# talha-alam/ADAM-Dehaze

Measured on AMD Instinct MI355X. Metric: images/sec CORUN-Complex fwd+bwd 512x1024 bs=8; PSNR vs CPU ref, higher is better.
Workload: dtype f32; 1 GPU; CORUN-Complex (HighIntensityDehazeModel base 96) train-mode fwd + L1 + bwd + Adam; per_gpu_batch=8, global_batch=8, height=512, width=1024, parallelism=dp1

## Files before the change

adam-dehaze_amd/csrc/conv_wino43.hip:

```cpp
#include "common.h"
#ifndef W_STORE_AUX
#define W_STORE_AUX 0
#endif
#include <cstdlib>
#include <type_traits>

#ifndef W4_DBG
#define W4_DBG 0
#endif
#ifndef W4_STORE_NOPS
#define W4_STORE_NOPS 1
#endif
#define W4_KC 16
#define W4_ZERO_C false
#define W4_TILES 32
#define W4_VF (36 * W4_TILES * W4_KC)
#define W4_SLOTS 612
#define W4_ROWSLOTS 34
#define W4_RAWF (40 * 256)
#define W4_TAB (W4_VF + W4_RAWF)
#define W4_TABF (4 * 640)
#define W4_MF (36 * 16 * 32)
#define W4_RED (W4_TAB + 3 * W4_TABF)
#define W4_LDS_BYTES ((W4_RED + 2 * 8 * 32) * 4)
static_assert(W4_MF <= W4_VF, "the epilogue's M must not reach the raw halo: the next region's first chunk lands there meanwhile");
#ifndef W4_P2
#define W4_P2 0
#endif
#define W4_PIECE_G0 2

#define W4B_RAW_B 73728
#define W4B_RAWBUF_B 40960
#define W4B_TAB_B 155648
#define W4B_LDS_BYTES (W4B_TAB_B + 3 * 2560)
static_assert(W4B_LDS_BYTES <= 160 * 1024, "LDS map of the bf16 x 3 variant");
#define B3_NO_SPLIT ((W4_DBG & 16) != 0)
#include "bf16x3.h"

typedef __attribute__((address_space(3))) void* lds_void_ptr4;

#ifdef W4_PROF
__device__ unsigned long long w4_prof_buf[16384 * 32];
#define W4_STAMP(i) do { if (tid == 0 && v < 16384) w4_prof_buf[v * 32 + (i)] = __builtin_readcyclecounter(); } while (0)
extern "C" int adh_w4_prof_read(void* dst) {
    return hipMemcpyFromSymbol(dst, HIP_SYMBOL(w4_prof_buf), sizeof(w4_prof_buf)) == hipSuccess ? 0 : -1;
}
#else
#define W4_STAMP(i) do {} while (0)
#endif

struct Wino43Geom {
    int tiles_x, tiles_y;
    int nregions;
    int nchunks;
    int KQtot;
    int ncog;
    int nvblocks;
    unsigned m_ncog, m_tx, m_ty;
    const float* bn_mean;
};

template <int NT, int FI, int J>
constexpr bool w4_in_agpr() {
    constexpr int nv = 9 * NT - 16;
    if constexpr (nv <= 0) return true;
    else if constexpr (nv <= 9) return !(J == 0 && FI >= 9 - nv);
    else return !(J == 0 || (J == 1 && FI >= 9 - (nv - 9)));
}
template <bool AGPR, bool Z = false>
__device__ __forceinline__ void w4_mfma(f32x16& c, float a, float b) {
    if constexpr (Z) {
        if constexpr (AGPR) asm("v_mfma_f32_32x32x2_f32 %0, %1, %2, 0" : "+a"(c) : "v"(a), "v"(b));
        else asm("v_mfma_f32_32x32x2_f32 %0, %1, %2, 0" : "+v"(c) : "v"(a), "v"(b));
    } else {
        if constexpr (AGPR) asm("v_mfma_f32_32x32x2_f32 %0, %1, %2, %0" : "+a"(c) : "v"(a), "v"(b));
        else asm("v_mfma_f32_32x32x2_f32 %0, %1, %2, %0" : "+v"(c) : "v"(a), "v"(b));
    }
}
#ifndef W4_MFMA_ZERO
#define W4_MFMA_ZERO 1
#endif
template <int NT, int T = 0>
__device__ __forceinline__ void w4_acc_zero_(f32x16 (&acc)[9 * NT], const u32x4& z) {
    if constexpr (T < 9 * NT) {
        if constexpr (w4_in_agpr<NT, T / NT, T % NT>()) asm volatile("v_mfma_f32_32x32x16_bf16 %0, %1, %1, 0" : "=a"(acc[T]) : "v"(z));
        else asm volatile("v_mfma_f32_32x32x16_bf16 %0, %1, %1, 0" : "=&v"(acc[T]) : "v"(z));
        w4_acc_zero_<NT, T + 1>(acc, z);
    }
}
template <int NT>
__device__ __forceinline__ void w4_acc_zero(f32x16 (&acc)[9 * NT]) {
    u32x4 z = {0u, 0u, 0u, 0u};
    asm volatile("s_nop 1" : "+v"(z));
    w4_acc_zero_<NT>(acc, z);
// ... 461 lines not shown
            in_next = image_ptr(wn.n);
            tab_nxt = tab_base;
            if (wn.border) {
                tab_nxt = tab_base + (1 + (tsel ^ 1)) * TABN;
                build_table(tab_nxt, wn.oy0, wn.ox0, false);
            }
        }
        W4_STAMP(4);
        const float* const b_wave = d.wp + ((int64_t)(wave * 9) * g.KQtot * d.NcP + co0) * 4;
        const char* const b3_wave = reinterpret_cast<const char*>(d.wp) + ((size_t)cg * g.nchunks * 36 + (size_t)wave * 9) * (NT * 3072);
        if constexpr (!BF3) {
            w4_load_b<NT>(bv[0], b_voff, b_wave);
            w4_load_b<NT>(bv[1], b_voff, b_wave + b_fstride);
        }
        W4_STAMP(5);
#if W4_MFMA_ZERO
        w4_acc_zero<NT>(acc);
#else
#pragma unroll
        for (int t = 0; t < 9 * NT; ++t)
#pragma unroll
            for (int r = 0; r < 16; ++r) acc[t][r] = 0.f;
#endif
        if (it == 0) asm volatile("s_waitcnt vmcnt(0)" ::: "memory");
        asm volatile("s_waitcnt lgkmcnt(0)" ::: "memory");
        __builtin_amdgcn_s_barrier();

        W4_STAMP(1);
#pragma unroll 1
        for (int c = 0; c < g.nchunks; ++c) {
            const bool more = c + 1 < g.nchunks;
            const bool cross = !more && has_next;
            st.cb = __builtin_amdgcn_readfirstlane((more ? (c + 1) * (W4_KC * 4) : (cross ? 0 : c * (W4_KC * 4))) + (cross ? wn.base : wc.base));
            st.rsrc = image_rsrc(cross ? in_next : in_cur);
            const int* const stab = cross ? tab_nxt : tab_cur;
            st.tab_lane = stab + tab_lane_o;
            if (c == 1) W4_STAMP(8);
            if (c == 1) W4_STAMP(9);
            if (!(W4_DBG & 1)) transform(cpar, stab);
            asm volatile("s_waitcnt lgkmcnt(0)" ::: "memory");
            if (c == 1) W4_STAMP(10);
            if constexpr (BF3) {
                if (!(W4_DBG & 2)) {
                    w4b_load_b(bv3[0], b3_voff, b3_wave + c * b3_cstride);
                    w4b_load_b(bv3[1], b3_voff, b3_wave + c * b3_cstride + 3072);
                }
            }
            __builtin_amdgcn_s_barrier();
            if (c == 1) W4_STAMP(11);
            if constexpr (BF3) {
                if (!(W4_DBG & 2)) {
                    w4b_load_s(nx, vlane, vlane1);
                    w4b_steps<0, 20>(nx, m1s);
                    av3[0] = u32x4{nx.h[0], nx.h[1], nx.h[2], nx.h[3]};
                    av3[1] = u32x4{nx.m[0], nx.m[1], nx.m[2], nx.m[3]};
                    av3[2] = u32x4{nx.l[0], nx.l[1], nx.l[2], nx.l[3]};
                    asm volatile("s_nop 1" : "+v"(av3[0]), "+v"(av3[1]), "+v"(av3[2]));
                    w4b_load_s(nx, vlane + W4_TILES * W4_KC, vlane1 + W4_TILES * W4_KC);
                    __builtin_amdgcn_sched_barrier(0);
                    w4b_groups<NT, 0, W4_ZERO_C>(acc, av3, nx, bv3, vlane, vlane1, b3_voff, b3_wave + c * b3_cstride, m1s);
                }
            } else if (!(W4_DBG & 2)) {
                const int cn = more ? c + 1 : c;
                const float* b_chunk = b_wave + (int64_t)(c * 4) * b_kq;
                const float* b_next = b_wave + (int64_t)(cn * 4) * b_kq;
                w4_contract<NT, W4_ZERO_C>(acc, av, bv, vlane, vlane1, b_voff, b_chunk, b_next, b_fstride, b_kq, st);
            }
            if (c == 1) W4_STAMP(12);
            cpar ^= 1;
            asm volatile("s_waitcnt lgkmcnt(0)" ::: "memory");
            __builtin_amdgcn_s_barrier();
            if (c == 1) W4_STAMP(13);
        }
        if constexpr (!BF3) {
            w4_wait_b<0, NT>(bv[0]);
            w4_wait_b<0, NT>(bv[1]);
        } else {
            asm volatile("s_waitcnt vmcnt(0)" ::: "memory");
        }
        W4_STAMP(2);

        if (!(W4_DBG & 4)) {
            float* M = lds;
            const int etp = (tid >> 3) & 15, eq = tid & 7;
            const int rh = wave >> 1;
            const int et = (etp & 8) | ((etp & 1) << 2) | ((etp >> 1) & 3);
            const int ey0 = oy0 + 4 * (et >> 3) + 2 * rh, ex0 = ox0 + 4 * (et & 7);
            float* out_n = d.out + (size_t)n * d.OH * d.OW * d.out_cstride;
            const float* res_n = d.residual ? d.residual + (size_t)n * d.OH * d.OW * d.res_cstride : nullptr;
            const int o_px = d.out_cstride * 4, o_row = d.OW * o_px;
            const int r_px = d.res_cstride * 4, r_row = d.OW * r_px;
            const __amdgpu_buffer_rsrc_t orsrc = __builtin_amdgcn_make_buffer_rsrc(out_n, 0, 0x7fffffff, 0x00020000);
            const __amdgpu_buffer_rsrc_t rrsrc =
                __builtin_amdgcn_make_buffer_rsrc(const_cast<float*>(res_n ? res_n : out_n), 0, 0x7fffffff, 0x00020000);
            const bool ragged = oy0 + 16 > d.OH || ox0 + 32 > d.OW;
            const float act_lo = d.act == ADH_ACT_RELU ? 0.f : -INFINITY;
            unsigned colpen[4];
#pragma unroll
            for (int r = 0; r < 4; ++r) colpen[r] = ex0 + r < d.OW ? 0u : 0x80000000u;
            const unsigned o_vbase = (unsigned)((ey0 * d.OW + ex0) * o_px + (co0 + eq * 4) * 4);
            const unsigned r_vbase = (unsigned)((ey0 * d.OW + ex0) * r_px + (co0 + eq * 4) * 4);
            const unsigned m_wbase = (unsigned)((wave * 9) * 2048 + h * 128 + l31 * 4);
            const float* const mp = M + etp * 32 + eq * 4;
            const float m1 = adh_opaque(-1.f);
            float* const red = BF3 ? lds + RAW0 + (cpar ^ 1) * (W4B_RAWBUF_B / 4) : lds + W4_RED;
            typedef unsigned u32x4 __attribute__((ext_vector_type(4)));
            w4_store_mh<NT, 0>(acc, m_wbase, 0);
            asm volatile("s_waitcnt lgkmcnt(0)" ::: "memory");
            __builtin_amdgcn_s_barrier();
#pragma unroll
            for (int j = 0; j < NT; ++j) {
                const int cq0 = co0 + j * 32 + eq * 4;
                const bool quad_ok = cq0 + 3 < d.Cout;
                f32x4 sc4 = {1.f, 1.f, 1.f, 1.f}, sh4 = {0.f, 0.f, 0.f, 0.f};
                if (d.scale && quad_ok) sc4 = *reinterpret_cast<const f32x4*>(d.scale + cq0);
                if (d.shift && quad_ok) sh4 = *reinterpret_cast<const f32x4*>(d.shift + cq0);
                f32x4 mean4 = {0.f, 0.f, 0.f, 0.f};
                if constexpr (BNRED) {
                    if (quad_ok) mean4 = *reinterpret_cast<const f32x4*>(g.bn_mean + cq0);
                }
                const unsigned chanpen = quad_ok ? 0u : 0x80000000u;
                const unsigned o_vj = (o_vbase + j * 128) | chanpen, r_vj = (r_vbase + j * 128) | chanpen;
                f32x4 ssum = {0.f, 0.f, 0.f, 0.f}, ssq = {0.f, 0.f, 0.f, 0.f};
#pragma unroll
                for (int th = 0; th < 2; ++th) {
                    if (j == 1 && th == 0) W4_STAMP(16);
                    f32x4 u[2][6];
#pragma unroll
                    for (int b = 0; b < 6; ++b) {
                        f32x4 m[6];
#pragma unroll
                        for (int a = 0; a < 6; ++a) m[a] = *reinterpret_cast<const f32x4*>(mp + (a * 6 + b) * (16 * 32));
                        const f32x4 s12 = m[1] + m[2], d12 = adh_pksub(m[1], m[2], m1), s34 = m[3] + m[4], d34 = adh_pksub(m[3], m[4], m1);
                        if (rh == 0) {
                            u[0][b] = m[0] + s12 + s34;
                            u[1][b] = W4_A * d12 + W4_B * d34;
                        } else {
                            u[0][b] = W4_A2 * s12 + W4_B2 * s34;
                            u[1][b] = W4_A3 * d12 + W4_B3 * d34 + m[5];
                        }
                    }
                    if (j == 1 && th == 0) W4_STAMP(17);
                    __builtin_amdgcn_s_barrier();
                    if (j == 1 && th == 0) W4_STAMP(18);
                    const int jn = th == 0 ? j : j + 1, thn = th ^ 1;
                    w4_store_mh_round<NT>(acc, m_wbase, jn, thn, 0);
                    if (j == 1 && th == 0) W4_STAMP(19);
                    unsigned rowpen[2];
#pragma unroll
                    for (int r = 0; r < 2; ++r) rowpen[r] = ey0 + 8 * th + r < d.OH ? 0u : 0x80000000u;
                    f32x4 rres[8];
                    if (res_n) {
#pragma unroll
                        for (int ii = 0; ii < 2; ++ii)
#pragma unroll
                            for (int jj = 0; jj < 4; ++jj)
                                rres[ii * 4 + jj] = __builtin_bit_cast(
                                    f32x4, __builtin_amdgcn_raw_buffer_load_b128(rrsrc, r_vj | rowpen[ii] | colpen[jj],
                                                                                 (8 * th + ii) * r_row + jj * r_px, 0));
                        asm volatile("" ::: "memory");
                    } else {
#pragma unroll
                        for (int q = 0; q < 8; ++q) rres[q] = f32x4{0.f, 0.f, 0.f, 0.f};
                    }
#pragma unroll
                    for (int ii = 0; ii < 2; ++ii) {
                        const f32x4 s12 = u[ii][1] + u[ii][2], d12 = adh_pksub(u[ii][1], u[ii][2], m1), s34 = u[ii][3] + u[ii][4],
                                    d34 = adh_pksub(u[ii][3], u[ii][4], m1);
                        const f32x4 y[4] = {u[ii][0] + s12 + s34, W4_A * d12 + W4_B * d34, W4_A2 * s12 + W4_B2 * s34,
                                            W4_A3 * d12 + W4_B3 * d34 + u[ii][5]};
#pragma unroll
                        for (int jj = 0; jj < 4; ++jj) {
                            const unsigned oaddr = o_vj | rowpen[ii] | colpen[jj];
                            if constexpr (BNRED) {
                                const f32x4 yv = rres[ii * 4 + jj];
                                const bool inside = (int)oaddr >= 0;
                                f32x4 gm;
#pragma unroll
                                for (int e = 0; e < 4; ++e) gm[e] = (inside && __builtin_fmaf(yv[e], sc4[e], sh4[e]) > 0.f) ? y[jj][e] : 0.f;
                                ssum += gm;
                                ssq += gm * adh_pksub(yv, mean4, m1);
                                f32x4 v4 = y[jj];
                                __builtin_amdgcn_raw_buffer_store_b128(__builtin_bit_cast(u32x4, v4), orsrc, oaddr,
                                                                       (8 * th + ii) * o_row + jj * o_px, W_STORE_AUX);
                                asm volatile("s_nop %1" : "+v"(v4) : "n"(W4_STORE_NOPS) : "memory");
                                w4_store_mh_round<NT>(acc, m_wbase, jn, thn, 1 + ii * 4 + jj);
                                continue;
                            }
                            f32x4 v4 = y[jj] * sc4 + sh4;
                            if (d.stats) {
                                f32x4 vs = v4;
                                if (ragged) {
                                    const bool inside = (int)oaddr >= 0;
#pragma unroll
                                    for (int e = 0; e < 4; ++e) vs[e] = inside ? v4[e] : 0.f;
                                    asm volatile("" : "+v"(vs));
                                }
                                ssum += vs;
                                ssq += vs * vs;
                            }
                            v4 += rres[ii * 4 + jj];
                            v4 = {fmaxf(v4[0], act_lo), fmaxf(v4[1], act_lo), fmaxf(v4[2], act_lo), fmaxf(v4[3], act_lo)};
                            __builtin_amdgcn_raw_buffer_store_b128(__builtin_bit_cast(u32x4, v4), orsrc, oaddr, (8 * th + ii) * o_row + jj * o_px,
                                                                   W_STORE_AUX);
                            asm volatile("s_nop %1" : "+v"(v4) : "n"(W4_STORE_NOPS) : "memory");
                            w4_store_mh_round<NT>(acc, m_wbase, jn, thn, 1 + ii * 4 + jj);
                        }
                    }
                    if (j == 1 && th == 0) W4_STAMP(20);
                    if (!(j == NT - 1 && th == 1)) {
                        asm volatile("s_waitcnt lgkmcnt(0)" ::: "memory");
                        __builtin_amdgcn_s_barrier();
                    }
                    if (j == 1 && th == 0) W4_STAMP(21);
                }
                if (d.stats) {
#pragma unroll
                    for (int e = 0; e < 4; ++e) {
#pragma unroll
                        for (int o = 8; o < 64; o <<= 1) {
                            ssum[e] += __shfl_xor(ssum[e], o, 64);
                            ssq[e] += __shfl_xor(ssq[e], o, 64);
                        }
                    }
// ... 287 lines not shown
```

adam-dehaze_amd/csrc/cbam.hip:

```cpp
#include "common.h"

#ifndef POOL_PPB
#define POOL_PPB 512
#endif
#ifndef CBAM_SCALE_MAXBLK
#define CBAM_SCALE_MAXBLK 65536
#endif
#ifndef CBAM_ROW_MAXBLK
#define CBAM_ROW_MAXBLK 2048
#endif

extern "C" int adh_cbam_pool_num_blocks(int HW) { return adh_ceil_div(HW, POOL_PPB); }

__global__ __launch_bounds__(256) void cbam_pool_partial_kernel(const float* __restrict__ x, int x_cs, int HW, int C,
                                                                float* __restrict__ partial,
                                                                int32_t* __restrict__ partial_idx, int nblk) {
    __shared__ f32x4 rs[256];
    __shared__ f32x4 rm[256];
    __shared__ int ri[256][4];
    const int n = blockIdx.y, blk = blockIdx.x;
    const int CQ = C / 4;
    const int R = 256 / CQ;
    const int cq = threadIdx.x % CQ, prow = threadIdx.x / CQ;
    const int c = cq * 4;
// ... 240 lines not shown
        sa[((size_t)n * H + y) * W + x] = 1.0f / (1.0f + expf(-v));
    }
}

__global__ __launch_bounds__(256) void cbam_scale_kernel(const float* __restrict__ x, int x_cs, const float* __restrict__ ca,
                                                         const float* __restrict__ sa, int64_t HW, int CQ,
                                                         float* __restrict__ out, int out_cs) {
    const int n = blockIdx.y;
    int64_t p, pstep;
    int c;
    adh_stream_decode(CQ, p, pstep, c);
    const f32x4 cav = *reinterpret_cast<const f32x4*>(ca + (size_t)n * CQ * 4 + c);
    const float* xn = x + (size_t)n * HW * x_cs;
    float* on = out + (size_t)n * HW * out_cs;
    const float* san = sa + (size_t)n * HW;
    for (; p < HW; p += 8 * pstep) {
        f32x4 v[8];
        float sv[8];
#pragma unroll
        for (int u = 0; u < 8; ++u) {
            const int64_t q = p + u * pstep < HW ? p + u * pstep : p;
            v[u] = __builtin_nontemporal_load(reinterpret_cast<const f32x4*>(xn + q * x_cs + c));
            sv[u] = san[q];
        }
#pragma unroll
        for (int u = 0; u < 8; ++u) {
            const int64_t q = p + u * pstep;
            if (q < HW) __builtin_nontemporal_store(v[u] * cav * sv[u], reinterpret_cast<f32x4*>(on + q * out_cs + c));
        }
    }
}

extern "C" int adh_cbam_apply(void* stream, const float* x, int x_cs, const float* ca, const float* smap,
                              const float* wsp, int N, int H, int W, int C, float* sa, float* out, int out_cs) {
    if (!x || !ca || !smap || !wsp || !sa || !out || N < 1 || H < 1 || W < 1 || C < 4 || (C & 3) || (x_cs & 3) || (out_cs & 3) ||
        N > 65535)
        return ADH_E_ARG;
    hipStream_t s = (hipStream_t)stream;
    hipLaunchKernelGGL(cbam_sa_kernel, dim3(adh_ceil_div(W, SA_TW), adh_ceil_div(H, SA_TH), N), dim3(256), 0, s, smap, wsp, H, W,
                       sa);
    hipLaunchKernelGGL(cbam_scale_kernel, dim3(adh_stream_blocks((int64_t)H * W, C / 4, 8, CBAM_SCALE_MAXBLK), N), dim3(256), 0, s,
                       x, x_cs, ca, sa, (int64_t)H * W, C / 4, out, out_cs);
    return adh_check_launch();
}

__global__ __launch_bounds__(256) void cbam_bwd_a_kernel(const float* __restrict__ g, int g_cs,
                                                         const float* __restrict__ x, int x_cs,
                                                         const float* __restrict__ ca, const float* __restrict__ sa,
                                                         int HW, int C, float* __restrict__ gsa_pre) {
    const int n = blockIdx.y;
    const int sub = threadIdx.x & 7;
    const int CQ = C / 4;
    const float* xn = x + (size_t)n * HW * x_cs;
    const float* gn = g + (size_t)n * HW * g_cs;
    const float* can = ca + (size_t)n * C;
    for (int p = blockIdx.x * 32 + (threadIdx.x >> 3); p < HW; p += gridDim.x * 32) {
        float s = 0.f;
        for (int q = sub; q < CQ; q += 8) {
            const f32x4 v = __builtin_nontemporal_load(reinterpret_cast<const f32x4*>(xn + (size_t)p * x_cs + q * 4)) *
                            *reinterpret_cast<const f32x4*>(can + q * 4) *
                            __builtin_nontemporal_load(reinterpret_cast<const f32x4*>(gn + (size_t)p * g_cs + q * 4));
            s += (v[0] + v[1]) + (v[2] + v[3]);
        }
#pragma unroll
        for (int o = 4; o > 0; o >>= 1) s += __shfl_xor(s, o, 64);
        if (sub == 0) {
            const float a = sa[(size_t)n * HW + p];
            gsa_pre[(size_t)n * HW + p] = s * a * (1.f - a);
        }
    }
}

extern "C" int adh_cbam_bwd_a(void* stream, const float* g, int g_cs, const float* x, int x_cs, const float* ca,
                              const float* sa, int N, int HW, int C, float* gsa_pre) {
    if (!g || !x || !ca || !sa || !gsa_pre || N < 1 || HW < 1 || C < 4 || (C & 3)) return ADH_E_ARG;
    const int blocks = adh_min_i(adh_ceil_div(HW, 32), CBAM_ROW_MAXBLK);
    hipLaunchKernelGGL(cbam_bwd_a_kernel, dim3(blocks, N), dim3(256), 0, (hipStream_t)stream, g, g_cs, x, x_cs, ca, sa, HW,
                       C, gsa_pre);
    return adh_check_launch();
}

extern "C" int adh_cbam_bwd_b_num_blocks(int N, int H, int W) { return adh_ceil_div((int64_t)N * H * W, 256); }

__global__ __launch_bounds__(256) void cbam_bwd_b_kernel(const float* __restrict__ gsa_pre,
                                                         const float* __restrict__ smap, const float* __restrict__ wsp,
                                                         int N, int H, int W, float* __restrict__ gsmap,
                                                         float* __restrict__ dwsp_partial) {
    __shared__ float s_w[98];
    __shared__ float s_acc[4][98];
    if (threadIdx.x < 98) s_w[threadIdx.x] = wsp[threadIdx.x];
    __syncthreads();
    const int64_t total = (int64_t)N * H * W;
    const int64_t idx = (int64_t)blockIdx.x * 256 + threadIdx.x;
    const bool valid = idx < total;
    int n = 0, y = 0, xx = 0;
    if (valid) {
        xx = (int)(idx % W);
        const int64_t r = idx / W;
        y = (int)(r % H);
        n = (int)(r / H);
    }
    const float* gp = gsa_pre + (size_t)n * H * W;
    const float* sm = smap + (size_t)n * H * W * 2;
    const float gs_here = valid ? gp[(size_t)y * W + xx] : 0.f;
    float g0 = 0.f, g1 = 0.f;
    const int wave = threadIdx.x >> 6, lane = threadIdx.x & 63;
    for (int ky = 0; ky < 7; ++ky) {
        for (int kx = 0; kx < 7; ++kx) {
            const int oy = y - ky + 3, ox = xx - kx + 3;
            if (valid && oy >= 0 && oy < H && ox >= 0 && ox < W) {
                const float go = gp[(size_t)oy * W + ox];
                g0 += go * s_w[ky * 7 + kx];
                g1 += go * s_w[49 + ky * 7 + kx];
            }
            const int iy = y + ky - 3, ix = xx + kx - 3;
            float a0 = 0.f, a1 = 0.f;
            if (valid && iy >= 0 && iy < H && ix >= 0 && ix < W) {
                const float* q = sm + ((size_t)iy * W + ix) * 2;
                a0 = q[0] * gs_here;
                a1 = q[1] * gs_here;
            }
            a0 = wave_sum(a0);
            a1 = wave_sum(a1);
            if (lane == 0) {
                s_acc[wave][ky * 7 + kx] = a0;
                s_acc[wave][49 + ky * 7 + kx] = a1;
            }
        }
    }
    if (valid) {
        gsmap[idx * 2 + 0] = g0;
        gsmap[idx * 2 + 1] = g1;
    }
    __syncthreads();
    if (threadIdx.x < 98)
        dwsp_partial[(size_t)blockIdx.x * 98 + threadIdx.x] =
            (s_acc[0][threadIdx.x] + s_acc[1][threadIdx.x]) + (s_acc[2][threadIdx.x] + s_acc[3][threadIdx.x]);
}

__global__ __launch_bounds__(256) void cbam_dwsp_final_kernel(const float* __restrict__ partial, int nblk, float* dwsp,
                                                              int accumulate) {
    __shared__ double red[256];
    const int o = blockIdx.x;
    double s = 0.0;
    for (int b = threadIdx.x; b < nblk; b += 256) s += (double)partial[(size_t)b * 98 + o];
    red[threadIdx.x] = s;
    __syncthreads();
    for (int st = 128; st > 0; st >>= 1) {
        if (threadIdx.x < st) red[threadIdx.x] += red[threadIdx.x + st];
        __syncthreads();
    }
    if (threadIdx.x == 0) dwsp[o] = accumulate ? dwsp[o] + (float)red[0] : (float)red[0];
}

extern "C" int adh_cbam_bwd_b(void* stream, const float* gsa_pre, const float* smap, const float* wsp, int N, int H,
                              int W, float* gsmap, float* dwsp_partial, int nblk, float* dwsp, int accumulate) {
    if (!gsa_pre || !smap || !wsp || !gsmap || !dwsp_partial || !dwsp) return ADH_E_ARG;
    if (nblk != adh_cbam_bwd_b_num_blocks(N, H, W)) return ADH_E_ARG;
    hipStream_t s = (hipStream_t)stream;
    hipLaunchKernelGGL(cbam_bwd_b_kernel, dim3(nblk), dim3(256), 0, s, gsa_pre, smap, wsp, N, H, W, gsmap, dwsp_partial);
    hipLaunchKernelGGL(cbam_dwsp_final_kernel, dim3(98), dim3(256), 0, s, dwsp_partial, nblk, dwsp, accumulate);
    return adh_check_launch();
}

__device__ __forceinline__ f32x4 cbam_gx1(const f32x4 g, float sa, float gmean_over_c, float gmax, int cidx, int c) {
    f32x4 r = g * sa + gmean_over_c;
#pragma unroll
    for (int j = 0; j < 4; ++j)
        if (c + j == cidx) r[j] += gmax;
    return r;
}

__global__ __launch_bounds__(256) void cbam_bwd_c_kernel(const float* __restrict__ g, int g_cs,
                                                         const float* __restrict__ x, int x_cs,
                                                         const float* __restrict__ sa, const float* __restrict__ gsmap,
                                                         const int32_t* __restrict__ cidx, int HW, int C,
                                                         float* __restrict__ gca_partial, int nblk) {
    __shared__ f32x4 rs[256];
    const int n = blockIdx.y, blk = blockIdx.x;
    const int CQ = C / 4;
    const int R = 256 / CQ;
    const int cq = threadIdx.x % CQ, prow = threadIdx.x / CQ;
    const int c = cq * 4;
    const float invC = 1.0f / (float)C;
    f32x4 s = {0.f, 0.f, 0.f, 0.f};
    if (prow < R) {
        const float* xn = x + (size_t)n * HW * x_cs;
        const float* gn = g + (size_t)n * HW * g_cs;
        const int p0 = blk * POOL_PPB;
        const int p1 = adh_min_i(p0 + POOL_PPB, HW);
        for (int p = p0 + prow; p < p1; p += 4 * R) {
            f32x4 gv[4], xv[4];
            float sv[4], gm[4], gx[4];
            int ci[4];
#pragma unroll
            for (int u = 0; u < 4; ++u) {
                const int q = p + u * R < p1 ? p + u * R : p;
                const size_t pp = (size_t)n * HW + q;
                gv[u] = __builtin_nontemporal_load(reinterpret_cast<const f32x4*>(gn + (size_t)q * g_cs + c));
                xv[u] = __builtin_nontemporal_load(reinterpret_cast<const f32x4*>(xn + (size_t)q * x_cs + c));
                sv[u] = sa[pp];
                gm[u] = gsmap[pp * 2 + 0];
                gx[u] = gsmap[pp * 2 + 1];
                ci[u] = cidx[pp];
            }
#pragma unroll
            for (int u = 0; u < 4; ++u)
                if (p + u * R < p1) s += cbam_gx1(gv[u], sv[u], gm[u] * invC, gx[u], ci[u], c) * xv[u];
        }
    }
    rs[threadIdx.x] = s;
    __syncthreads();
    if (threadIdx.x < CQ) {
        f32x4 S = {0.f, 0.f, 0.f, 0.f};
        for (int r = 0; r < R; ++r) S += rs[r * CQ + threadIdx.x];
        *reinterpret_cast<f32x4*>(gca_partial + ((size_t)n * nblk + blk) * C + c) = S;
    }
}

extern "C" int adh_cbam_bwd_c(void* stream, const float* g, int g_cs, const float* x, int x_cs, const float* sa,
                              const float* gsmap, const int32_t* cidx, int N, int HW, int C, float* gca_partial,
                              int nblk) {
    if (!g || !x || !sa || !gsmap || !cidx || !gca_partial || C < 4 || (C & 3) || C > 1024) return ADH_E_ARG;
    if (nblk != adh_cbam_pool_num_blocks(HW)) return ADH_E_ARG;
    hipLaunchKernelGGL(cbam_bwd_c_kernel, dim3(nblk, N), dim3(256), 0, (hipStream_t)stream, g, g_cs, x, x_cs, sa, gsmap,
                       cidx, HW, C, gca_partial, nblk);
    return adh_check_launch();
}

__global__ __launch_bounds__(256) void cbam_bwd_d1_kernel(const float* __restrict__ gca_partial, int nblk,
                                                          const float* __restrict__ ca, int C, float* __restrict__ gpre) {
    __shared__ double red[8][32];
    const int n = blockIdx.y;
    const int cl = threadIdx.x & 31, grp = threadIdx.x >> 5;
    const int c = blockIdx.x * 32 + cl;
    double s = 0.0;
    if (c < C)
        for (int b = grp; b < nblk; b += 8) s += (double)gca_partial[((size_t)n * nblk + b) * C + c];
    red[grp][cl] = s;
    __syncthreads();
    if (grp == 0 && c < C) {
// ... 145 lines not shown
```

adam-dehaze_amd/csrc/conv_wgrad.hip:

```cpp
#include "common.h"
#include <cstdlib>

#define WG_TW 32

template <int T, int TN>
__global__ __launch_bounds__(512, 2) void conv_wgrad_kernel(const adh_conv_desc d, const ConvGeom g, float* slab,
                                                            int ntiles, int KP, int nco_groups) {
    extern __shared__ __attribute__((aligned(16))) float smem[];
    constexpr int BN = 32 * TN;
    constexpr int PER = (T * TN + 3) / 4;
    const int XP = g.xp;
    const int buf_floats = g.npx * XP + 32 + g.TH * WG_TW * BN;

    const int tid = threadIdx.x;
    const int lane = tid & 63;
    const int wave = __builtin_amdgcn_readfirstlane(tid >> 6);
    const bool loader = wave >= 4;
    const int l31 = lane & 31;
    const int h = lane >> 5;

    const int ci_tile = blockIdx.x / nco_groups;
    const int co_grp = blockIdx.x - ci_tile * nco_groups;
    const int ci0 = ci_tile * 32;
    const int co0 = co_grp * BN;
// ... 528 lines not shown
                p.a.xps = 2;
                p.a.ymin = d->dy0 + py;
                p.a.xmin = d->dx0 + px;
                p.a.tap0 = py * 4 + px; p.a.tap_sy = 8; p.a.tap_sx = 2;
            }
        return 4;
    }
    return 0;
}

template <int KH, int KW, bool REV, int TN>
static int launch_wgrad_rows(hipStream_t s, const adh_conv_desc* d, const WrArgs& a, float* slab) {
    const int lds = 2 * (((WR_TH + KH - 1) * WR_HP + TN * WR_TH * 32) * 32 * 4);
    const int nblocks = adh_split_grid_blocks(a.nsplit, a.ngroups);
    (void)hipFuncSetAttribute(reinterpret_cast<const void*>(&conv_wgrad_rows_kernel<KH, KW, REV, TN>),
                              hipFuncAttributeMaxDynamicSharedMemorySize, 160 * 1024);
    hipLaunchKernelGGL((conv_wgrad_rows_kernel<KH, KW, REV, TN>), dim3(nblocks), dim3(256), lds, s, *d, a, slab);
    return adh_check_launch();
}

static int dispatch_wgrad_rows(hipStream_t s, const adh_conv_desc* d, const WrPlan& p, float* slab) {
#define WR_CASE(kh_, kw_, rev_, tn_) \
    if (p.KH == kh_ && p.KW == kw_ && p.rev == rev_ && p.TN == tn_) \
        return launch_wgrad_rows<kh_, kw_, rev_ != 0, tn_>(s, d, p.a, slab);
    WR_CASE(3, 3, 0, 3) WR_CASE(3, 3, 0, 2) WR_CASE(3, 3, 0, 1)
    WR_CASE(2, 2, 0, 3) WR_CASE(2, 2, 0, 2) WR_CASE(2, 2, 0, 1)
    WR_CASE(2, 2, 1, 3) WR_CASE(2, 2, 1, 2) WR_CASE(2, 2, 1, 1)
#undef WR_CASE
    return ADH_E_UNSUPPORTED;
}

static bool wgrad_rows_instantiated(const WrPlan& p) {
    return (p.KH == 3 && p.KW == 3 && !p.rev) || (p.KH == 2 && p.KW == 2);
}

static int wgrad_wino_plan(const adh_conv_desc* d, int nsplit, WrPlan* p) {
    static const bool enabled = !(getenv("ADH_WINO_WGRAD") && atoi(getenv("ADH_WINO_WGRAD")) == 0);
    if (!enabled) return 0;
    WrPlan plan[4];
    if (wgrad_rows_plan(d, nsplit, plan) != 1) return 0;
    if (plan[0].KH != 3 || plan[0].KW != 3 || plan[0].rev || plan[0].a.xps != 1) return 0;
    if (d->dy0 != -1 || d->dx0 != -1) return 0;
    *p = plan[0];
    return 1;
}

extern "C" int adh_conv_wgrad_wino_groups(const adh_conv_desc* d) {
    if (!d) return ADH_E_ARG;
    WrPlan p;
    return wgrad_wino_plan(d, 1, &p) ? p.a.ngroups : 0;
}

extern "C" int adh_conv_wgrad_wino(void* stream, const adh_conv_desc* d, float* slab, int nsplit) {
    if (!d || !slab || nsplit < 1 || !d->in || !d->out) return ADH_E_ARG;
    WrPlan p;
    if (!wgrad_wino_plan(d, nsplit, &p)) return ADH_E_UNSUPPORTED;
    const int lds = 2 * (((WR_TH + 2) * WR_HP + p.TN * WR_TH * 32) * 32 * 4);
    const int nblocks = adh_split_grid_blocks(nsplit, p.a.ngroups);
    hipStream_t s = (hipStream_t)stream;
#define WW_CASE(tn_) \
    if (p.TN == tn_) { \
        (void)hipFuncSetAttribute(reinterpret_cast<const void*>(&conv_wgrad_rows_kernel<3, 3, false, tn_, true>), \
                                  hipFuncAttributeMaxDynamicSharedMemorySize, 160 * 1024); \
        hipLaunchKernelGGL((conv_wgrad_rows_kernel<3, 3, false, tn_, true>), dim3(nblocks), dim3(256), lds, s, *d, p.a, slab); \
        return adh_check_launch(); \
    }
    WW_CASE(3) WW_CASE(2) WW_CASE(1)
#undef WW_CASE
    return ADH_E_UNSUPPORTED;
}

extern "C" int adh_conv_wgrad_groups(const adh_conv_desc* d) {
    if (!d) return ADH_E_ARG;
    WrPlan plan[4];
    const int n = wgrad_rows_plan(d, 1, plan);
    return n && wgrad_rows_instantiated(plan[0]) ? plan[0].a.ngroups : 0;
}

extern "C" int adh_conv_wgrad_slabs(const adh_conv_desc* d, int nsplit) {
    if (!d || nsplit < 1) return ADH_E_ARG;
    return adh_conv_wgrad_groups(d) > 0 ? 4 * nsplit : nsplit;
}

extern "C" int adh_conv_wgrad(void* stream, const adh_conv_desc* d, float* slab, int nsplit) {
    if (!d || !slab || nsplit < 1 || !d->in || !d->out) return ADH_E_ARG;
    if (d->NcP % 32 != 0 || d->NcP < d->Cout) return ADH_E_ARG;
    {
        WrPlan plan[4];
        const int np = wgrad_rows_plan(d, nsplit, plan);
        if (np && wgrad_rows_instantiated(plan[0])) {
            for (int i = 0; i < np; ++i) {
                const int rc = dispatch_wgrad_rows((hipStream_t)stream, d, plan[i], slab);
                if (rc) return rc;
            }
            return ADH_OK;
        }
    }
    const int Ttot = d->KH * d->KW;
    int T;
    if (Ttot == 9 || Ttot == 16 || Ttot == 4 || Ttot == 1) T = Ttot;
    else if (Ttot == 49 || Ttot == 14) T = 7;
    else return ADH_E_UNSUPPORTED;
    const bool packed = (d->dstep_x == 4 && d->Cin == 8 && d->in_sx == 1);
    const int TN = wgrad_pick_tn(d->NcP, T);
    ConvGeom g;
    int rc = wgrad_geometry(d, &g, TN, packed ? 8 : 32);
    if (rc) return rc;
    if ((d->VH - 1) * d->out_sy + d->out_oy >= d->OH || (d->VW - 1) * d->out_sx + d->out_ox >= d->OW) return ADH_E_ARG;
    const int KP = adh_round_up(d->Cin, 32);
    hipStream_t s = (hipStream_t)stream;
#define WG_CASE(t, tn) \
    if (T == t && TN == tn) { launch_wgrad<t, tn>(s, d, g, slab, nsplit, KP); return adh_check_launch(); }
    WG_CASE(9, 4) WG_CASE(9, 3) WG_CASE(9, 2) WG_CASE(9, 1)
    WG_CASE(16, 3) WG_CASE(16, 2) WG_CASE(16, 1)
    WG_CASE(4, 4) WG_CASE(4, 3) WG_CASE(4, 2) WG_CASE(4, 1)
    WG_CASE(7, 4) WG_CASE(7, 3) WG_CASE(7, 2) WG_CASE(7, 1)
    WG_CASE(1, 4) WG_CASE(1, 3) WG_CASE(1, 2) WG_CASE(1, 1)
#undef WG_CASE
    return ADH_E_UNSUPPORTED;
}
```

Before: 40.38 images/sec.

## Split Winograd epilogue row transform across lane halves with permlane32 swap

Remaps the Winograd F(4,3) output-transform epilogue so each wave's lane halves each read half of the M columns (3 of 6) from LDS. Each lane computes all four output-row combinations for its columns, then exchanges results across the 32-lane halves with permlane32_swap, instead of every lane reading all six columns and computing only its two rows. This aims to halve LDS reads and remove the rh-dependent branching in the epilogue. The cost is extra cross-lane swap instructions, changed LDS write and read addressing, and a dependency on a lane_rebuilt helper for the BF3 path.

```diff
diff --git a/adam-dehaze_amd/csrc/conv_wino43.hip b/adam-dehaze_amd/csrc/conv_wino43.hip
--- a/adam-dehaze_amd/csrc/conv_wino43.hip
+++ b/adam-dehaze_amd/csrc/conv_wino43.hip
@@ -10,6 +10,9 @@
 #endif
 #ifndef W4_STORE_NOPS
 #define W4_STORE_NOPS 1
+#endif
+#ifndef W4_EPI_PAIR
+#define W4_EPI_PAIR 1
 #endif
 #define W4_KC 16
 #define W4_ZERO_C false
@@ -637,8 +640,14 @@
 
         if (!(W4_DBG & 4)) {
             float* M = lds;
+#if W4_EPI_PAIR
+            const int eln = BF3 ? lane_rebuilt() : lane;
+            const int etp = (wave << 2) | ((eln >> 3) & 3), eq = eln & 7;
+            const int rh = eln >> 5;
+#else
             const int etp = (tid >> 3) & 15, eq = tid & 7;
             const int rh = wave >> 1;
+#endif
             const int et = (etp & 8) | ((etp & 1) << 2) | ((etp >> 1) & 3);
             const int ey0 = oy0 + 4 * (et >> 3) + 2 * rh, ex0 = ox0 + 4 * (et & 7);
             float* out_n = d.out + (size_t)n * d.OH * d.OW * d.out_cstride;
@@ -655,8 +664,12 @@
             for (int r = 0; r < 4; ++r) colpen[r] = ex0 + r < d.OW ? 0u : 0x80000000u;
             const unsigned o_vbase = (unsigned)((ey0 * d.OW + ex0) * o_px + (co0 + eq * 4) * 4);
             const unsigned r_vbase = (unsigned)((ey0 * d.OW + ex0) * r_px + (co0 + eq * 4) * 4);
+#if W4_EPI_PAIR
+            const unsigned m_wbase = (unsigned)((wave * 9) * 2048 + eln * 4);
+#else
             const unsigned m_wbase = (unsigned)((wave * 9) * 2048 + h * 128 + l31 * 4);
-            const float* const mp = M + etp * 32 + eq * 4;
+#endif
+            const float* const mp = M + etp * 32 + eq * 4 + (W4_EPI_PAIR ? rh * (3 * 16 * 32) : 0);
             const float m1 = adh_opaque(-1.f);
             float* const red = BF3 ? lds + RAW0 + (cpar ^ 1) * (W4B_RAWBUF_B / 4) : lds + W4_RED;
             typedef unsigned u32x4 __attribute__((ext_vector_type(4)));
@@ -681,6 +694,35 @@
                 for (int th = 0; th < 2; ++th) {
                     if (j == 1 && th == 0) W4_STAMP(16);
                     f32x4 u[2][6];
+#if W4_EPI_PAIR
+                    {
+                        f32x4 t[4][3];
+#pragma unroll
+                        for (int k = 0; k < 3; ++k) {
+                            f32x4 m[6];
+#pragma unroll
+                            for (int a = 0; a < 6; ++a) m[a] = *reinterpret_cast<const f32x4*>(mp + (a * 6 + k) * (16 * 32));
+                            const f32x4 s12 = m[1] + m[2], d12 = adh_pksub(m[1], m[2], m1), s34 = m[3] + m[4], d34 = adh_pksub(m[3], m[4], m1);
+                            t[0][k] = m[0] + s12 + s34;
+                            t[1][k] = W4_A * d12 + W4_B * d34;
+                            t[2][k] = W4_A2 * s12 + W4_B2 * s34;
+                            t[3][k] = W4_A3 * d12 + W4_B3 * d34 + m[5];
+                        }
+#pragma unroll
+                        for (int k = 0; k < 3; ++k)
+#pragma unroll
+                            for (int ii = 0; ii < 2; ++ii) {
+#pragma unroll
+                                for (int e = 0; e < 4; ++e) {
+                                    const float lo = t[ii][k][e], hi = t[2 + ii][k][e];
+                                    const auto r = __builtin_amdgcn_permlane32_swap(__float_as_uint(lo), __float_as_uint(hi), false, false);
+                                    const unsigned r0 = r[0], r1 = r[1];
+                                    u[ii][k][e] = __uint_as_float(r0);
+                                    u[ii][3 + k][e] = __uint_as_float(r1);
+                                }
+                            }
+                    }
+#else
 #pragma unroll
                     for (int b = 0; b < 6; ++b) {
                         f32x4 m[6];
@@ -695,6 +737,7 @@
                             u[1][b] = W4_A3 * d12 + W4_B3 * d34 + m[5];
                         }
                     }
+#endif
                     if (j == 1 && th == 0) W4_STAMP(17);
                     __builtin_amdgcn_s_barrier();
                     if (j == 1 && th == 0) W4_STAMP(18);
```

Result: no change. 40.57 images/sec (median of 6 runs) (+0.5%).

## Stage CBAM spatial-backward halo in LDS and add dedicated 1x1 head wgrad kernel

Applied to the files above, without the earlier changes.

The CBAM spatial-attention backward kernel now loads a 7-row halo of gsa_pre and the 2-channel pooled map into shared memory once per block. It then computes the 7x7 input gradient and the weight-gradient partials from LDS, replacing the per-tap wave reductions with a transposed shared-memory reduction done once per kernel row. A separate specialised wgrad kernel handles the 1x1 head conv (Cin=16, Cout<=4) as a streaming reduction with nontemporal vector loads instead of the generic tiled wgrad path. Both changes target memory-bound small kernels and add shape and alignment guards, and more syncthreads in the CBAM path.

```diff
diff --git a/adam-dehaze_amd/csrc/cbam.hip b/adam-dehaze_amd/csrc/cbam.hip
--- a/adam-dehaze_amd/csrc/cbam.hip
+++ b/adam-dehaze_amd/csrc/cbam.hip
@@ -346,60 +346,102 @@
 
 extern "C" int adh_cbam_bwd_b_num_blocks(int N, int H, int W) { return adh_ceil_div((int64_t)N * H * W, 256); }
 
+typedef float cbam_f32x2 __attribute__((vector_size(8)));
+#define CBAM_B_RUN 262
+#define CBAM_B_PITCH 264
+#define CBAM_B_WPITCH 68
+#define CBAM_B_TPITCH (4 * CBAM_B_WPITCH)
+
 __global__ __launch_bounds__(256) void cbam_bwd_b_kernel(const float* __restrict__ gsa_pre,
                                                          const float* __restrict__ smap, const float* __restrict__ wsp,
                                                          int N, int H, int W, float* __restrict__ gsmap,
                                                          float* __restrict__ dwsp_partial) {
     __shared__ float s_w[98];
-    __shared__ float s_acc[4][98];
-    if (threadIdx.x < 98) s_w[threadIdx.x] = wsp[threadIdx.x];
-    __syncthreads();
+    __shared__ float s_g[7 * CBAM_B_PITCH];
+    __shared__ cbam_f32x2 s_sm[7 * CBAM_B_PITCH];
+    __shared__ float s_t[14 * CBAM_B_TPITCH];
+    static_assert(7 * CBAM_B_PITCH >= 98 * 16, "s_g holds the last stage");
+    const int t = threadIdx.x;
+    if (t < 98) s_w[t] = wsp[t];
     const int64_t total = (int64_t)N * H * W;
-    const int64_t idx = (int64_t)blockIdx.x * 256 + threadIdx.x;
+    const int64_t base = (int64_t)blockIdx.x * 256;
+    const cbam_f32x2* sm2 = reinterpret_cast<const cbam_f32x2*>(smap);
+    for (int e = t; e < 7 * CBAM_B_RUN; e += 256) {
+        const int r = e / CBAM_B_RUN, i = e - r * CBAM_B_RUN;
+        const int64_t q = base + (int64_t)(r - 3) * W - 3 + i;
+        const bool in = q >= 0 && q < total;
+        const cbam_f32x2 zero = {0.f, 0.f};
+        s_g[r * CBAM_B_PITCH + i] = in ? gsa_pre[q] : 0.f;
+        s_sm[r * CBAM_B_PITCH + i] = in ? sm2[q] : zero;
+    }
+    __syncthreads();
+    const int64_t idx = base + t;
     const bool valid = idx < total;
-    int n = 0, y = 0, xx = 0;
+    int y = 0, xx = 0;
     if (valid) {
         xx = (int)(idx % W);
-        const int64_t r = idx / W;
-        y = (int)(r % H);
-        n = (int)(r / H);
-    }
-    const float* gp = gsa_pre + (size_t)n * H * W;
-    const float* sm = smap + (size_t)n * H * W * 2;
-    const float gs_here = valid ? gp[(size_t)y * W + xx] : 0.f;
+        y = (int)((idx / W) % H);
+    }
+    const float gs_here = s_g[3 * CBAM_B_PITCH + t + 3];
     float g0 = 0.f, g1 = 0.f;
-    const int wave = threadIdx.x >> 6, lane = threadIdx.x & 63;
+    const int wave = t >> 6, lane = t & 63;
+    const int jj = t >> 4, aw = (t >> 2) & 3, ai = t & 3;
+    float acc[7];
+#pragma unroll
     for (int ky = 0; ky < 7; ++ky) {
+        const int oy = y - ky + 3;
+        const bool oy_in = valid && oy >= 0 && oy < H;
+        const int iy = y + ky - 3;
+        const bool iy_in = valid && iy >= 0 && iy < H;
+#pragma unroll
         for (int kx = 0; kx < 7; ++kx) {
-            const int oy = y - ky + 3, ox = xx - kx + 3;
-            if (valid && oy >= 0 && oy < H && ox >= 0 && ox < W) {
-                const float go = gp[(size_t)oy * W + ox];
+            const int ox = xx - kx + 3;
+            if (oy_in && ox >= 0 && ox < W) {
+                const float go = s_g[(6 - ky) * CBAM_B_PITCH + t + 6 - kx];
                 g0 += go * s_w[ky * 7 + kx];
                 g1 += go * s_w[49 + ky * 7 + kx];
             }
-            const int iy = y + ky - 3, ix = xx + kx - 3;
+            const int ix = xx + kx - 3;
             float a0 = 0.f, a1 = 0.f;
-            if (valid && iy >= 0 && iy < H && ix >= 0 && ix < W) {
-                const float* q = sm + ((size_t)iy * W + ix) * 2;
+            if (iy_in && ix >= 0 && ix < W) {
+                const cbam_f32x2 q = s_sm[ky * CBAM_B_PITCH + t + kx];
                 a0 = q[0] * gs_here;
                 a1 = q[1] * gs_here;
             }
-            a0 = wave_sum(a0);
-            a1 = wave_sum(a1);
-            if (lane == 0) {
-                s_acc[wave][ky * 7 + kx] = a0;
-                s_acc[wave][49 + ky * 7 + kx] = a1;
-            }
-        }
+            s_t[kx * CBAM_B_TPITCH + wave * CBAM_B_WPITCH + lane] = a0;
+            s_t[(7 + kx) * CBAM_B_TPITCH + wave * CBAM_B_WPITCH + lane] = a1;
+        }
+        __syncthreads();
+        float r = 0.f;
+        if (jj < 14) {
+            const float* v = s_t + jj * CBAM_B_TPITCH + aw * CBAM_B_WPITCH + ai;
+            float a[8];
+#pragma unroll
+            for (int k = 0; k < 8; ++k) a[k] = v[4 * k] + v[4 * (k + 8)];
+#pragma unroll
+            for (int k = 0; k < 4; ++k) a[k] += a[k + 4];
+            r = (a[0] + a[2]) + (a[1] + a[3]);
+        }
+        acc[ky] = r;
+        __syncthreads();
     }
     if (valid) {
         gsmap[idx * 2 + 0] = g0;
         gsmap[idx * 2 + 1] = g1;
     }
-    __syncthreads();
-    if (threadIdx.x < 98)
-        dwsp_partial[(size_t)blockIdx.x * 98 + threadIdx.x] =
-            (s_acc[0][threadIdx.x] + s_acc[1][threadIdx.x]) + (s_acc[2][threadIdx.x] + s_acc[3][threadIdx.x]);
+    if (jj < 14) {
+        const int ch = jj / 7, kx = jj - ch * 7;
+#pragma unroll
+        for (int ky = 0; ky < 7; ++ky) s_g[(ch * 49 + ky * 7 + kx) * 16 + aw * 4 + ai] = acc[ky];
+    }
+    __syncthreads();
+    if (t < 98) {
+        const float* v = s_g + t * 16;
+        float w[4];
+#pragma unroll
+        for (int k = 0; k < 4; ++k) w[k] = (v[4 * k] + v[4 * k + 2]) + (v[4 * k + 1] + v[4 * k + 3]);
+        dwsp_partial[(size_t)blockIdx.x * 98 + t] = (w[0] + w[1]) + (w[2] + w[3]);
+    }
 }
 
 __global__ __launch_bounds__(256) void cbam_dwsp_final_kernel(const float* __restrict__ partial, int nblk, float* dwsp,
@@ -421,6 +463,7 @@
                               int W, float* gsmap, float* dwsp_partial, int nblk, float* dwsp, int accumulate) {
     if (!gsa_pre || !smap || !wsp || !gsmap || !dwsp_partial || !dwsp) return ADH_E_ARG;
     if (nblk != adh_cbam_bwd_b_num_blocks(N, H, W)) return ADH_E_ARG;
+    if ((uintptr_t)smap & 7) return ADH_E_ARG;
     hipStream_t s = (hipStream_t)stream;
     hipLaunchKernelGGL(cbam_bwd_b_kernel, dim3(nblk), dim3(256), 0, s, gsa_pre, smap, wsp, N, H, W, gsmap, dwsp_partial);
     hipLaunchKernelGGL(cbam_dwsp_final_kernel, dim3(98), dim3(256), 0, s, dwsp_partial, nblk, dwsp, accumulate);
diff --git a/adam-dehaze_amd/csrc/conv_wgrad.hip b/adam-dehaze_amd/csrc/conv_wgrad.hip
--- a/adam-dehaze_amd/csrc/conv_wgrad.hip
+++ b/adam-dehaze_amd/csrc/conv_wgrad.hip
@@ -634,9 +634,72 @@
     return adh_conv_wgrad_groups(d) > 0 ? 4 * nsplit : nsplit;
 }
 
+#define WG1_UNROLL 8
+__global__ __launch_bounds__(256) void conv_wgrad_head1x1_kernel(const float* __restrict__ x, int x_cs,
+                                                                 const float* __restrict__ g, int g_cs, int64_t P,
+                                                                 int Cout, float* __restrict__ slab, int KP, int NcP) {
+    __shared__ f32x4 red[4][4][4];
+    const int q = threadIdx.x & 3, slot = threadIdx.x >> 2;
+    const int64_t per = (P + gridDim.x - 1) / gridDim.x;
+    const int64_t p0 = (int64_t)blockIdx.x * per;
+    const int64_t p1 = p0 + per < P ? p0 + per : P;
+    f32x4 acc[4];
+#pragma unroll
+    for (int co = 0; co < 4; ++co) acc[co] = f32x4{0.f, 0.f, 0.f, 0.f};
+    for (int64_t p = p0 + slot; p < p1; p += 64 * WG1_UNROLL) {
+        f32x4 xv[WG1_UNROLL], gv[WG1_UNROLL];
+#pragma unroll
+        for (int u = 0; u < WG1_UNROLL; ++u) {
+            const int64_t pp = p + 64 * u;
+            xv[u] = f32x4{0.f, 0.f, 0.f, 0.f};
+            gv[u] = f32x4{0.f, 0.f, 0.f, 0.f};
+            if (pp < p1) {
+                xv[u] = __builtin_nontemporal_load(reinterpret_cast<const f32x4*>(x + pp * x_cs + q * 4));
+                gv[u] = __builtin_nontemporal_load(reinterpret_cast<const f32x4*>(g + pp * g_cs));
+            }
+        }
+#pragma unroll
+        for (int u = 0; u < WG1_UNROLL; ++u)
+#pragma unroll
+            for (int co = 0; co < 4; ++co) acc[co] += xv[u] * gv[u][co];
+    }
+#pragma unroll
+    for (int o = 4; o < 64; o <<= 1)
+#pragma unroll
+        for (int co = 0; co < 4; ++co)
+#pragma unroll
+            for (int j = 0; j < 4; ++j) acc[co][j] += __shfl_xor(acc[co][j], o, 64);
+    if ((threadIdx.x & 63) < 4) {
+#pragma unroll
+        for (int co = 0; co < 4; ++co) red[threadIdx.x >> 6][co][q] = acc[co];
+    }
+    __syncthreads();
+    float* const sl = slab + (size_t)blockIdx.x * KP * NcP;
+    for (int i = threadIdx.x; i < KP * NcP; i += 256) {
+        const int ci = i / NcP, co = i - ci * NcP;
+        float v = 0.f;
+        if (co < Cout && ci < 16)
+            v = (red[0][co][ci >> 2][ci & 3] + red[1][co][ci >> 2][ci & 3]) + (red[2][co][ci >> 2][ci & 3] + red[3][co][ci >> 2][ci & 3]);
+        sl[i] = v;
+    }
+}
+
+static bool wgrad_head1x1_shape(const adh_conv_desc* d) {
+    return d->KH == 1 && d->KW == 1 && d->Cin == 16 && d->Cout >= 1 && d->Cout <= 4 && d->in_cstride >= 16 &&
+           d->in_cstride % 4 == 0 && d->out_cstride >= 4 && d->out_cstride % 4 == 0 && !((uintptr_t)d->in & 15) &&
+           !((uintptr_t)d->out & 15) && d->in_sy == 1 && d->in_sx == 1 && d->out_sy == 1 &&
+           d->out_sx == 1 && d->out_oy == 0 && d->out_ox == 0 && d->dy0 == 0 && d->dx0 == 0 && d->VH == d->IH &&
+           d->VW == d->IW && d->VH == d->OH && d->VW == d->OW;
+}
+
 extern "C" int adh_conv_wgrad(void* stream, const adh_conv_desc* d, float* slab, int nsplit) {
     if (!d || !slab || nsplit < 1 || !d->in || !d->out) return ADH_E_ARG;
     if (d->NcP % 32 != 0 || d->NcP < d->Cout) return ADH_E_ARG;
+    if (wgrad_head1x1_shape(d)) {
+        hipLaunchKernelGGL(conv_wgrad_head1x1_kernel, dim3(nsplit), dim3(256), 0, (hipStream_t)stream, d->in, d->in_cstride,
+                           d->out, d->out_cstride, (int64_t)d->N * d->VH * d->VW, d->Cout, slab, 32, d->NcP);
+        return adh_check_launch();
+    }
     {
         WrPlan plan[4];
         const int np = wgrad_rows_plan(d, nsplit, plan);
```

Measured after the change: 40.41 images/sec before, 40.55 images/sec after (median of 6 runs). About the same (+0.4%).
